# nurturenature/jepsen-tigerbeetle

Measured on AMD Instinct MI355X. Metric: histories/sec, 10k-op/64-proc cas-register histories (time-to-verdict ms in extra), higher is better.
Workload: dtype u64

## Files before the change

jepsen-tigerbeetle_amd/csrc/open_walk_impl.h:

```cpp
#pragma once
#include "wave_env.h"
#include "tbc_internal.h"

namespace tbc {
namespace walk {

constexpr uint32_t kCandCap = 136;
constexpr uint32_t kCandWords = 8;
constexpr uint32_t kAuxWords = 80;
WV_HD constexpr uint32_t walk_lds_words() { return kCandCap * kCandWords + kAuxWords; }

constexpr uint32_t kCList = 1u;
constexpr uint32_t kCTwin = 2u;
constexpr uint32_t kCRow = 4u;
constexpr uint32_t kCLook = 8u;

WV_DEV void or_slot(uint32_t& lo, uint32_t& hi, bool cond, uint32_t slot) {
  if (slot < 32u) lo = wv::opaque(lo | (cond ? (1u << slot) : 0u));
  else hi = wv::opaque(hi | (cond ? (1u << (slot - 32u)) : 0u));
}
WV_DEV uint32_t effect_key(uint32_t f, int32_t a, int32_t b) {
  return (f & 3u) | (((uint32_t)a & 0x7FFFu) << 2) | ((f == TBC_F_CAS ? ((uint32_t)b & 0x7FFFu) : 0u) << 17);
}
static_assert(kMaxRuleValue < 0x7FFF && TBC_F_READ < 3 && TBC_F_WRITE < 3 && TBC_F_CAS < 3, "effect_key packs f and two rule values into a word, and no key has all bits set");
static_assert(kLookNone <= 0xFFu, "the produced value shares a word with the flags");

WV_DEV uint32_t rank_code(uint32_t slot, uint32_t f, int32_t a, uint32_t vpad) {
  const uint32_t k8 = f == TBC_F_READ ? (rdm_index(a, vpad) & 0xFFu) : 0xFFu;
  return (slot & 63u) | ((k8 == 0xFFu ? 7u : (k8 & 7u)) << 6);
}

template <int Q>
WV_DEV void store_entries(const wv::u32x16& r, uint64_t* row, uint32_t n) {
  WV_UNROLL
  for (int v = 0; v < 8; v++) if ((uint32_t)(8 * Q + v) < n) row[8 * Q + v] = (uint64_t)r[2 * v] | ((uint64_t)r[2 * v + 1] << 32);
}

template <int VCAP>
WV_DEV void walk_wave(const PackOpenArgs& A, uint32_t wid, uint32_t* lds, uint32_t lane) {
  const uint32_t cph = A.chunks_per_hist;
  const uint32_t hr = wid / cph, c = wid - hr * cph, h = A.h0 + hr;
  if (h >= A.n_hist) return;
  const Hist* H = &A.hist[h];
  const BeamHist* B = &A.bh[h];
  const uint32_t R = H->n_ret;
  const uint32_t F_lo = c * 64u;
  if (H->status != 0 || B->status != 0 || F_lo >= R) return;
  const uint32_t F_hi = F_lo + 64u < R ? F_lo + 64u : R;
  const uint32_t W = H->n_slots;
  const Rec* rec = A.rec + H->rec_off;
  const uint32_t* seg = A.seg + H->seg_off;
  const uint32_t* off = A.off + B->off_off;
  OpRec* lst = A.lst + B->lst_off;
  uint64_t* twn = A.twn ? A.twn + B->lst_off : nullptr;
  const uint32_t V = A.vpad;
  const uint32_t FW = A.front_words ? A.front_words : V;
  const bool compact = A.front_compact != 0u;
  uint64_t* rdm = (A.rdm && (V || compact)) ? A.rdm + H->op_off * FW : nullptr;
  const bool want_tw = twn != nullptr;
  uint64_t* look = A.look ? A.look + look_off(H->op_off, h, 1u) : nullptr;
  uint32_t* cand = lds;
  uint32_t* aux = lds + kCandCap * kCandWords;

  const uint32_t ret_from = look ? (F_lo >= kLookahead - 1u ? F_lo - (kLookahead - 1u) : 0u) : F_lo;
  uint32_t lo = 0, k = 0;
  if (lane < W) {
    uint32_t l = seg[lane] + 1u, hi = seg[lane + 1] - 1u;
    const uint32_t tail = hi;
    while (l < hi) {
      const uint32_t mid = (l + hi) >> 1;
      if (rec[mid].ret_rank >= ret_from) hi = mid; else l = mid + 1u;
    }
    lo = l;
    uint32_t i = lo;
    for (;;) {
      const uint32_t i1 = i + 1u < tail ? i + 1u : tail, i2 = i + 2u < tail ? i + 2u : tail, i3 = i + 3u < tail ? i + 3u : tail;
      const uint32_t v0 = rec[i < tail ? i : tail].inv_rank, v1 = rec[i1].inv_rank, v2 = rec[i2].inv_rank, v3 = rec[i3].inv_rank;
      if (v0 >= F_hi) break;
      i++;
      if (v1 >= F_hi) break;
      i++;
      if (v2 >= F_hi) break;
      i++;
      if (v3 >= F_hi) break;
      i++;
    }
    k = i - lo;
  }
  uint32_t incl = k;
  for (uint32_t d = 1; d < 64u; d <<= 1) {
    aux[lane] = incl;
    wv::barrier();
    const uint32_t add = lane >= d ? aux[lane - d] : 0u;
    wv::barrier();
    incl += add;
  }
  const uint32_t base = incl - k;
  const uint32_t NC_all = wv::readlane(incl, 63u);
  const uint32_t NC = NC_all < kCandCap ? NC_all : kCandCap;
  for (uint32_t j = 0; j < k; j++) {
    const Rec r = rec[lo + j];
    if (base + j < kCandCap) {
      const bool live = (r.cls & 2u) != 0u, isread = (r.cls & 16u) != 0u, wc = (r.cls & 8u) != 0u;
      const bool in_chunk = r.ret_rank >= F_lo;
      const bool listed = live && in_chunk && !(A.branch_lists && isread);
      const uint32_t vi = rdm_index(r.a, V);
      uint32_t fl = (lane << 12) | (r.prod << 24);
      if (listed) fl |= kCList;
      if (listed && wc && want_tw) fl |= kCTwin;
      if (live && in_chunk && isread && rdm && V && (vi != 0u || r.a == TBC_NIL)) fl |= kCRow | (vi << 4);
      if (look && (r.cls & 6u) && r.prod != kLookNone) fl |= kCLook;
      uint32_t* e = cand + (base + j) * kCandWords;
      e[0] = r.inv_rank; e[1] = r.ret_rank; e[2] = r.opidx; e[3] = r.f | (lane << 8);
      e[4] = (uint32_t)r.a; e[5] = (uint32_t)r.b; e[6] = fl;
      e[7] = (live && wc && in_chunk) ? effect_key(r.f, r.a, r.b) : 0xFFFFFFFFu;
    }
  }
  wv::barrier();

  const uint32_t list_order = A.order_of ? A.order_of[h] : A.list_order;
  const bool by_ret = list_order != 0u;
  const uint32_t wr_last = list_order == 2u ? 0x40000000u : list_order >= 16u ? 2u * (list_order - 16u) + 1u : 0u;
  const uint32_t rk_mul = list_order >= 16u ? 2u : 1u;
  uint16_t* const perm = reinterpret_cast<uint16_t*>(aux);
  if (by_ret) {
    uint32_t my[3], place[3] = {0u, 0u, 0u};
    WV_UNROLL
    for (int s = 0; s < 3; s++) {
      const uint32_t idx = lane + 64u * (uint32_t)s;
      const uint32_t* e = cand + (idx < NC ? idx : 0u) * kCandWords;
      const uint32_t rt = e[1];
      my[s] = idx >= NC ? 0xFFFFFFFFu : rt == kInf ? (0xFFFFFF00u | idx) : rt * rk_mul + ((e[3] & 0xFFu) == TBC_F_WRITE ? wr_last : 0u);
    }
    const uint32_t n0 = NC < 64u ? NC : 64u, n1 = NC <= 64u ? 0u : (NC < 128u ? NC - 64u : 64u), n2 = NC <= 128u ? 0u : NC - 128u;
    if (NC <= 64u) {
      for (uint32_t j = 0; j < n0; j++) place[0] += wv::readlane(my[0], j) < my[0] ? 1u : 0u;
    } else if (NC <= 128u) {
      for (uint32_t j = 0; j < n0; j++) { const uint32_t kj = wv::readlane(my[0], j); place[0] += kj < my[0] ? 1u : 0u; place[1] += kj < my[1] ? 1u : 0u; }
      for (uint32_t j = 0; j < n1; j++) { const uint32_t kj = wv::readlane(my[1], j); place[0] += kj < my[0] ? 1u : 0u; place[1] += kj < my[1] ? 1u : 0u; }
    } else {
      WV_UNROLL
      for (int s2 = 0; s2 < 3; s2++) {
        const uint32_t cnt = s2 == 0 ? n0 : s2 == 1 ? n1 : n2;
        for (uint32_t j = 0; j < cnt; j++) {
          const uint32_t kj = wv::readlane(my[s2], j);
          place[0] += kj < my[0] ? 1u : 0u; place[1] += kj < my[1] ? 1u : 0u; place[2] += kj < my[2] ? 1u : 0u;
        }
      }
    }
    WV_UNROLL
    for (int s = 0; s < 3; s++) {
      const uint32_t idx = lane + 64u * (uint32_t)s;
      if (idx < NC) perm[place[s]] = (uint16_t)idx;
    }
    wv::barrier();
  }

  uint32_t c_key[3] = {0xFFFFFFFFu, 0xFFFFFFFFu, 0xFFFFFFFFu}, c_ret[3] = {0u, 0u, 0u};
  if (want_tw) {
    WV_UNROLL
    for (int s = 0; s < 3; s++) {
      const uint32_t idx = lane + 64u * (uint32_t)s;
      const uint32_t* e = cand + (idx < NC ? idx : 0u) * kCandWords;
      c_key[s] = idx < NC ? e[7] : 0xFFFFFFFFu;
      c_ret[s] = e[1];
    }
  }

  const uint32_t F = F_lo + lane;
  const bool active = F < F_hi;
  const uint32_t Fc = active ? F : F_hi - 1u;
  const uint32_t pos0 = off[Fc];
  uint32_t pos = pos0;
  const uint32_t px = A.ret_slot[H->ret_off + Fc];
  uint32_t need = kLookNone, xprod = kLookNone, di = 0, x = 0, xf = kFNone;
  int32_t xa = 0;
  if (look || compact) {
    x = A.ret_op[H->ret_off + Fc];
    xf = A.f[H->op_off + x];
    xa = A.a[H->op_off + x];
  }
  if (look) {
    const int32_t xb = A.b[H->op_off + x];
    const uint32_t xinv = A.scratch[H->frame_off + x];
    need = look_need(xf, xa); xprod = look_prod(xf, xa, xb);
    di = F - xinv < 255u ? F - xinv : 255u;
  }
  wv::u32x16 r0, r1, r2, r3;
  WV_UNROLL
  for (int i = 0; i < 16; i++) { r0[i] = 0u; r1[i] = 0u; r2[i] = 0u; r3[i] = 0u; }
  uint32_t pm_lo = 0u, pm_hi = 0u, dmin = 255u;

  WV_NOUNROLL
  for (uint32_t t = 0; t < NC; t++) {
    const uint32_t* e = cand + (by_ret ? (uint32_t)perm[t] : t) * kCandWords;
    const uint32_t inv = e[0], ret = e[1];
    const uint32_t fl = wv::readfirstlane(e[6]);
    const uint32_t slot = (fl >> 12) & 63u;
    const bool member = active && inv <= F && F <= ret;
    if (fl & kCList) {
      uint32_t tw_lo = 0u, tw_hi = 0u;
      if (fl & kCTwin) {
        const uint32_t key_t = e[7];
        uint64_t s0 = wv::ballot(c_key[0] == key_t && c_ret[0] < ret && c_ret[0] >= inv);
        uint64_t s1 = 0ull, s2 = 0ull;
        if (NC > 64u) s1 = wv::ballot(c_key[1] == key_t && c_ret[1] < ret && c_ret[1] >= inv);
        if (NC > 128u) s2 = wv::ballot(c_key[2] == key_t && c_ret[2] < ret && c_ret[2] >= inv);
        while (s0 | s1 | s2) {
          uint32_t u;
          if (s0) { u = (uint32_t)__builtin_ctzll(s0); s0 &= s0 - 1ull; }
          else if (s1) { u = 64u + (uint32_t)__builtin_ctzll(s1); s1 &= s1 - 1ull; }
          else { u = 128u + (uint32_t)__builtin_ctzll(s2); s2 &= s2 - 1ull; }
          const uint32_t* eu = cand + u * kCandWords;
          const bool mu = eu[0] <= F && F <= eu[1];
          or_slot(tw_lo, tw_hi, mu, (wv::readfirstlane(eu[6]) >> 12) & 63u);
        }
      }
      if (member) {
        OpRec o; o.op = e[2]; o.f_slot = e[3] | (ret == F ? kAtFront : 0u); o.a = (int32_t)e[4]; o.b = (int32_t)e[5];
        lst[pos] = o;
        if (twn) twn[pos] = (uint64_t)tw_lo | ((uint64_t)tw_hi << 32);
        pos++;
      }
    }
    if (fl & kCRow)
    {
      const uint32_t w = ((fl >> 4) & 31u) * 2u + (slot >> 5), bit = member ? (1u << (slot & 31u)) : 0u;
      if constexpr (VCAP <= 8) r0[w & 15u] |= bit;
      else {
        const uint32_t q = w >> 4;
        if (q == 0u) r0[w & 15u] |= bit; else if (q == 1u) r1[w & 15u] |= bit; else if (q == 2u) r2[w & 15u] |= bit; else r3[w & 15u] |= bit;
      }
    }
    if (fl & kCLook) {
      const bool hit = (fl >> 24) == need;
      or_slot(pm_lo, pm_hi, member && hit, slot);
      const uint32_t dist = F - inv;
      if (hit && dist < kLookahead && e[2] != x) dmin = dist < dmin ? dist : dmin;
    }
  }

  uint64_t w6 = 0ull, w7 = 0ull;
  if (compact) {
    if (by_ret) wv::barrier();
    aux[lane] = active ? rank_code(px, xf, xa, V) : (7u << 6);
    if (lane < kFrontCompactRanks - 1u) {
      const uint32_t G = F_lo + 64u + lane;
      uint32_t code = 7u << 6;
      if (G < R) {
        const uint32_t gx = A.ret_op[H->ret_off + G];
        code = rank_code(A.ret_slot[H->ret_off + G], A.f[H->op_off + gx], A.a[H->op_off + gx], V);
      }
      aux[64u + lane] = code;
    }
    wv::barrier();
    WV_UNROLL
    for (uint32_t l = 0; l < kFrontCompactRanks; l++) w7 |= (uint64_t)aux[lane + l] << (9u * l);
    const uint32_t nl = pos - pos0, nc = A.ncr[B->off_off + Fc];
    w6 = (uint64_t)pos0 | ((uint64_t)(nl & 0xFFu) << 32) | ((uint64_t)((nl + nc) & 0xFFFFFFu) << 40);
  }
  if (!active) return;
  if (rdm) {
    uint64_t* row = rdm + (uint64_t)F * FW;
    const uint32_t n_row = compact ? 6u : V;
    store_entries<0>(r0, row, n_row);
    if constexpr (VCAP > 8) { store_entries<1>(r1, row, n_row); store_entries<2>(r2, row, n_row); store_entries<3>(r3, row, n_row); }
    if (compact) { row[6] = w6; row[7] = w7; }
  }
  if (look) {
    uint64_t pm = (uint64_t)pm_lo | ((uint64_t)pm_hi << 32);
    pm &= ~(1ull << (px & 63u));
    const uint64_t w0 = (uint64_t)(px & 0xFFFFu) | (uint64_t)need << 16 | (uint64_t)xprod << 24 | (uint64_t)di << 32 | ((uint64_t)dmin << 40);
    look[(uint64_t)F * 2u] = w0;
    look[(uint64_t)F * 2u + 1u] = pm;
  }
}

}
}
```

Measured before the change: 379,900.

## Physically sort walk candidates in LDS and split twin/list emission into second pass

Candidates in LDS are reordered in place by return rank, using 16-byte moves, instead of being reached through a uint16 permutation. The entry layout changes so the hot fields (inv, ret, key, flags) sit in the first 16 bytes. The main walk loop now only records per-lane membership bitmasks and marks candidates that have any twin. A second pass emits list entries and computes twin masks only for the marked candidates, scanning the member bits. This removes an indirection and the per-candidate serial twin scan from the wave-uniform loop, at the cost of extra barriers, LDS writes of flags, and a divergent per-lane emission loop.

Measured after the change: 382,300 (median of 4 runs). No clear change (+0.6%).

```diff
diff --git a/jepsen-tigerbeetle_amd/csrc/open_walk_impl.h b/jepsen-tigerbeetle_amd/csrc/open_walk_impl.h
--- a/jepsen-tigerbeetle_amd/csrc/open_walk_impl.h
+++ b/jepsen-tigerbeetle_amd/csrc/open_walk_impl.h
@@ -8,12 +8,14 @@
 constexpr uint32_t kCandCap = 136;
 constexpr uint32_t kCandWords = 8;
 constexpr uint32_t kAuxWords = 80;
+static_assert((kCandCap * kCandWords + kAuxWords) % 4u == 0u, "a wavefront's candidates are read 16 bytes at a time");
 WV_HD constexpr uint32_t walk_lds_words() { return kCandCap * kCandWords + kAuxWords; }
 
 constexpr uint32_t kCList = 1u;
 constexpr uint32_t kCTwin = 2u;
 constexpr uint32_t kCRow = 4u;
 constexpr uint32_t kCLook = 8u;
+constexpr uint32_t kCHasTwin = 1u << 18;
 
 WV_DEV void or_slot(uint32_t& lo, uint32_t& hi, bool cond, uint32_t slot) {
   if (slot < 32u) lo = wv::opaque(lo | (cond ? (1u << slot) : 0u));
@@ -23,6 +25,7 @@
   return (f & 3u) | (((uint32_t)a & 0x7FFFu) << 2) | ((f == TBC_F_CAS ? ((uint32_t)b & 0x7FFFu) : 0u) << 17);
 }
 static_assert(kMaxRuleValue < 0x7FFF && TBC_F_READ < 3 && TBC_F_WRITE < 3 && TBC_F_CAS < 3, "effect_key packs f and two rule values into a word, and no key has all bits set");
+static_assert(kAtFront == 1u << 31, "the member loop shifts the flag into place");
 static_assert(kLookNone <= 0xFFu, "the produced value shares a word with the flags");
 
 WV_DEV uint32_t rank_code(uint32_t slot, uint32_t f, int32_t a, uint32_t vpad) {
@@ -111,9 +114,9 @@
       if (live && in_chunk && isread && rdm && V && (vi != 0u || r.a == TBC_NIL)) fl |= kCRow | (vi << 4);
       if (look && (r.cls & 6u) && r.prod != kLookNone) fl |= kCLook;
       uint32_t* e = cand + (base + j) * kCandWords;
-      e[0] = r.inv_rank; e[1] = r.ret_rank; e[2] = r.opidx; e[3] = r.f | (lane << 8);
-      e[4] = (uint32_t)r.a; e[5] = (uint32_t)r.b; e[6] = fl;
-      e[7] = (live && wc && in_chunk) ? effect_key(r.f, r.a, r.b) : 0xFFFFFFFFu;
+      e[0] = r.inv_rank; e[1] = r.ret_rank; e[3] = fl;
+      e[2] = (live && wc && in_chunk) ? effect_key(r.f, r.a, r.b) : 0xFFFFFFFFu;
+      e[4] = r.opidx; e[5] = r.f | (lane << 8); e[6] = (uint32_t)r.a; e[7] = (uint32_t)r.b;
     }
   }
   wv::barrier();
@@ -122,7 +125,6 @@
   const bool by_ret = list_order != 0u;
   const uint32_t wr_last = list_order == 2u ? 0x40000000u : list_order >= 16u ? 2u * (list_order - 16u) + 1u : 0u;
   const uint32_t rk_mul = list_order >= 16u ? 2u : 1u;
-  uint16_t* const perm = reinterpret_cast<uint16_t*>(aux);
   if (by_ret) {
     uint32_t my[3], place[3] = {0u, 0u, 0u};
     WV_UNROLL
@@ -130,7 +132,7 @@
       const uint32_t idx = lane + 64u * (uint32_t)s;
       const uint32_t* e = cand + (idx < NC ? idx : 0u) * kCandWords;
       const uint32_t rt = e[1];
-      my[s] = idx >= NC ? 0xFFFFFFFFu : rt == kInf ? (0xFFFFFF00u | idx) : rt * rk_mul + ((e[3] & 0xFFu) == TBC_F_WRITE ? wr_last : 0u);
+      my[s] = idx >= NC ? 0xFFFFFFFFu : rt == kInf ? (0xFFFFFF00u | idx) : rt * rk_mul + ((e[5] & 0xFFu) == TBC_F_WRITE ? wr_last : 0u);
     }
     const uint32_t n0 = NC < 64u ? NC : 64u, n1 = NC <= 64u ? 0u : (NC < 128u ? NC - 64u : 64u), n2 = NC <= 128u ? 0u : NC - 128u;
     if (NC <= 64u) {
@@ -148,10 +150,23 @@
         }
       }
     }
+    wv::u32x4 mv[3][2] = {};
     WV_UNROLL
     for (int s = 0; s < 3; s++) {
       const uint32_t idx = lane + 64u * (uint32_t)s;
-      if (idx < NC) perm[place[s]] = (uint16_t)idx;
+      if (idx < NC) {
+        const wv::u32x4* e4 = reinterpret_cast<const wv::u32x4*>(cand + idx * kCandWords);
+        mv[s][0] = e4[0]; mv[s][1] = e4[1];
+      }
+    }
+    wv::barrier();
+    WV_UNROLL
+    for (int s = 0; s < 3; s++) {
+      const uint32_t idx = lane + 64u * (uint32_t)s;
+      if (idx < NC) {
+        wv::u32x4* e4 = reinterpret_cast<wv::u32x4*>(cand + place[s] * kCandWords);
+        e4[0] = mv[s][0]; e4[1] = mv[s][1];
+      }
     }
     wv::barrier();
   }
@@ -162,7 +177,7 @@
     for (int s = 0; s < 3; s++) {
       const uint32_t idx = lane + 64u * (uint32_t)s;
       const uint32_t* e = cand + (idx < NC ? idx : 0u) * kCandWords;
-      c_key[s] = idx < NC ? e[7] : 0xFFFFFFFFu;
+      c_key[s] = idx < NC ? e[2] : 0xFFFFFFFFu;
       c_ret[s] = e[1];
     }
   }
@@ -186,64 +201,89 @@
     need = look_need(xf, xa); xprod = look_prod(xf, xa, xb);
     di = F - xinv < 255u ? F - xinv : 255u;
   }
+  const uint32_t w0_lo = wv::opaque((px & 0xFFFFu) | need << 16 | xprod << 24), my_code = wv::opaque(rank_code(px, xf, xa, V));
   wv::u32x16 r0, r1, r2, r3;
   WV_UNROLL
   for (int i = 0; i < 16; i++) { r0[i] = 0u; r1[i] = 0u; r2[i] = 0u; r3[i] = 0u; }
   uint32_t pm_lo = 0u, pm_hi = 0u, dmin = 255u;
 
+  uint32_t m0 = 0u, m1 = 0u, m2 = 0u, m3 = 0u, m4 = 0u;
   WV_NOUNROLL
-  for (uint32_t t = 0; t < NC; t++) {
-    const uint32_t* e = cand + (by_ret ? (uint32_t)perm[t] : t) * kCandWords;
-    const uint32_t inv = e[0], ret = e[1];
-    const uint32_t fl = wv::readfirstlane(e[6]);
-    const uint32_t slot = (fl >> 12) & 63u;
-    const bool member = active && inv <= F && F <= ret;
-    if (fl & kCList) {
-      uint32_t tw_lo = 0u, tw_hi = 0u;
-      if (fl & kCTwin) {
-        const uint32_t key_t = e[7];
-        uint64_t s0 = wv::ballot(c_key[0] == key_t && c_ret[0] < ret && c_ret[0] >= inv);
-        uint64_t s1 = 0ull, s2 = 0ull;
-        if (NC > 64u) s1 = wv::ballot(c_key[1] == key_t && c_ret[1] < ret && c_ret[1] >= inv);
-        if (NC > 128u) s2 = wv::ballot(c_key[2] == key_t && c_ret[2] < ret && c_ret[2] >= inv);
-        while (s0 | s1 | s2) {
-          uint32_t u;
-          if (s0) { u = (uint32_t)__builtin_ctzll(s0); s0 &= s0 - 1ull; }
-          else if (s1) { u = 64u + (uint32_t)__builtin_ctzll(s1); s1 &= s1 - 1ull; }
-          else { u = 128u + (uint32_t)__builtin_ctzll(s2); s2 &= s2 - 1ull; }
-          const uint32_t* eu = cand + u * kCandWords;
-          const bool mu = eu[0] <= F && F <= eu[1];
-          or_slot(tw_lo, tw_hi, mu, (wv::readfirstlane(eu[6]) >> 12) & 63u);
+  for (uint32_t tw0 = 0; tw0 < NC; tw0 += 32u) {
+    const uint32_t t_end = tw0 + 32u < NC ? tw0 + 32u : NC;
+    uint32_t m = 0u;
+    WV_NOUNROLL
+    for (uint32_t t = tw0; t < t_end; t++) {
+      uint32_t* e = cand + t * kCandWords;
+      const uint32_t inv = e[0], ret = e[1];
+      const uint32_t fl = wv::readfirstlane(e[3]);
+      const uint32_t slot = (fl >> 12) & 63u;
+      const bool member = active && inv <= F && F <= ret;
+      if (fl & kCList) {
+        m |= member ? (1u << (t & 31u)) : 0u;
+        if (fl & kCTwin) {
+          const uint32_t key_t = e[2];
+          uint64_t s_any = wv::ballot(c_key[0] == key_t && c_ret[0] < ret && c_ret[0] >= inv);
+          if (NC > 64u) s_any |= wv::ballot(c_key[1] == key_t && c_ret[1] < ret && c_ret[1] >= inv);
+          if (NC > 128u) s_any |= wv::ballot(c_key[2] == key_t && c_ret[2] < ret && c_ret[2] >= inv);
+          if (s_any != 0ull && lane == 0u) e[3] = fl | kCHasTwin;
         }
       }
-      if (member) {
-        OpRec o; o.op = e[2]; o.f_slot = e[3] | (ret == F ? kAtFront : 0u); o.a = (int32_t)e[4]; o.b = (int32_t)e[5];
-        lst[pos] = o;
-        if (twn) twn[pos] = (uint64_t)tw_lo | ((uint64_t)tw_hi << 32);
-        pos++;
-      }
-    }
-    if (fl & kCRow)
-    {
-      const uint32_t w = ((fl >> 4) & 31u) * 2u + (slot >> 5), bit = member ? (1u << (slot & 31u)) : 0u;
-      if constexpr (VCAP <= 8) r0[w & 15u] |= bit;
-      else {
-        const uint32_t q = w >> 4;
-        if (q == 0u) r0[w & 15u] |= bit; else if (q == 1u) r1[w & 15u] |= bit; else if (q == 2u) r2[w & 15u] |= bit; else r3[w & 15u] |= bit;
-      }
-    }
-    if (fl & kCLook) {
-      const bool hit = (fl >> 24) == need;
-      or_slot(pm_lo, pm_hi, member && hit, slot);
-      const uint32_t dist = F - inv;
-      if (hit && dist < kLookahead && e[2] != x) dmin = dist < dmin ? dist : dmin;
+      if (fl & kCRow)
+      {
+        const uint32_t w = ((fl >> 4) & 31u) * 2u + (slot >> 5), bit = member ? (1u << (slot & 31u)) : 0u;
+        if constexpr (VCAP <= 8) r0[w & 15u] |= bit;
+        else {
+          const uint32_t q = w >> 4;
+          if (q == 0u) r0[w & 15u] |= bit; else if (q == 1u) r1[w & 15u] |= bit; else if (q == 2u) r2[w & 15u] |= bit; else r3[w & 15u] |= bit;
+        }
+      }
+      if (fl & kCLook) {
+        const bool hit = (fl >> 24) == need;
+        or_slot(pm_lo, pm_hi, member && hit, slot);
+        const uint32_t dist = F - inv;
+        if (hit && dist < kLookahead && ret != F) dmin = dist < dmin ? dist : dmin;
+      }
+    }
+    const uint32_t wq = tw0 >> 5;
+    if (wq == 0u) m0 = m; else if (wq == 1u) m1 = m; else if (wq == 2u) m2 = m; else if (wq == 3u) m3 = m; else m4 = m;
+  }
+  wv::barrier();
+
+  {
+    const uint64_t all_a = (uint64_t)m0 | ((uint64_t)m1 << 32), all_b = (uint64_t)m2 | ((uint64_t)m3 << 32);
+    const uint32_t all_c = m4;
+    uint64_t qa = all_a, qb = all_b;
+    uint32_t qc = all_c, qbase = 0u;
+    while ((qa | qb | (uint64_t)qc) != 0ull) {
+      while (qa == 0ull) { qa = qb; qb = (uint64_t)qc; qc = 0u; qbase += 64u; }
+      const uint32_t p = qbase + (uint32_t)__builtin_ctzll(qa);
+      qa &= qa - 1ull;
+      const uint32_t* e = cand + p * kCandWords;
+      const uint32_t ret_t = e[1], key_t = e[2], fl_t = e[3];
+      const wv::u32x4 h1 = *reinterpret_cast<const wv::u32x4*>(e + 4);
+      uint64_t tw = 0ull;
+      if (fl_t & kCHasTwin) {
+        auto scan = [&](uint64_t x, uint32_t xbase) {
+          while (x != 0ull) {
+            const uint32_t q = xbase + (uint32_t)__builtin_ctzll(x);
+            x &= x - 1ull;
+            const uint32_t* eu = cand + q * kCandWords;
+            if (eu[2] == key_t && eu[1] < ret_t) tw |= 1ull << ((eu[3] >> 12) & 63u);
+          }
+        };
+        scan(all_a, 0u); scan(all_b, 64u); scan((uint64_t)all_c, 128u);
+      }
+      OpRec o; o.op = h1.x; o.f_slot = h1.y | ((ret_t == F ? 1u : 0u) << 31); o.a = (int32_t)h1.z; o.b = (int32_t)h1.w;
+      lst[pos] = o;
+      if (twn) twn[pos] = tw;
+      pos++;
     }
   }
 
   uint64_t w6 = 0ull, w7 = 0ull;
   if (compact) {
-    if (by_ret) wv::barrier();
-    aux[lane] = active ? rank_code(px, xf, xa, V) : (7u << 6);
+    aux[lane] = active ? my_code : (7u << 6);
     if (lane < kFrontCompactRanks - 1u) {
       const uint32_t G = F_lo + 64u + lane;
       uint32_t code = 7u << 6;
@@ -269,8 +309,8 @@
   }
   if (look) {
     uint64_t pm = (uint64_t)pm_lo | ((uint64_t)pm_hi << 32);
-    pm &= ~(1ull << (px & 63u));
-    const uint64_t w0 = (uint64_t)(px & 0xFFFFu) | (uint64_t)need << 16 | (uint64_t)xprod << 24 | (uint64_t)di << 32 | ((uint64_t)dmin << 40);
+    pm &= ~(1ull << (w0_lo & 63u));
+    const uint64_t w0 = (uint64_t)w0_lo | (uint64_t)di << 32 | ((uint64_t)dmin << 40);
     look[(uint64_t)F * 2u] = w0;
     look[(uint64_t)F * 2u + 1u] = pm;
   }
```
